# Lacadame/DiffSci

Measured on AMD Instinct MI355X. Metric: samples/sec (50-step Karras Heun), PUNetG 64ch 128x128, higher is better.
Workload: dtype f32 (3x3 convs: fp16 hi+lo split, 3 fp16 MFMA products, fp32 accumulate); 1 GPU; PUNetG 64-base-ch, 1x128x128 fields, batch 64 per GPU, 50-step Heun deterministic sampler (99 network evaluations); global_batch=64, parallelism=dp1 (batch shards, all-gather of samples), world_size=1, backend=none (one process), hipgraph=True

## Files before the change

diffsci_amd/csrc/ds_attn3h.hip:

```cpp
#include <cstdlib>

#include "ds_common.h"
#include "ds_conv_epilogue.h"
#include "ds_h3_common.h"

namespace {

using ds::f32x4;
using ds::wave_max;
using ds_epi::f32x16;
using ds_h3::f16x8;
using ds_h3::split2;
using ds_h3::u32x4;
typedef unsigned u32x2 __attribute__((ext_vector_type(2)));

constexpr int NT = 256;
constexpr int KB = 32;
constexpr float RESCALE_T = 8.0f;

constexpr float LOG2E = 1.44269504088896341f;

__device__ __forceinline__ f16x8 as_f16x8(u32x4 v) { return __builtin_bit_cast(f16x8, v); }

template <int ET, bool IMG, bool MH>
__global__ __launch_bounds__(NT) void k_attn3h(float* out, const float* __restrict__ q, size_t q_bs,
                                               const u32x4* __restrict__ kimg, const u32x4* __restrict__ vimg, int L, int heads,
                                               float scale, float thr, const unsigned* q_amax, const unsigned* k_amax,
                                               const unsigned* v_amax, unsigned* out_amax) {
  constexpr int E = 32 * ET;
  constexpr int NDG = E / 8;
  constexpr int NS = E / 16;
  constexpr int KITEMS = NDG * KB;
  constexpr int KI = (KITEMS + NT - 1) / NT;
  constexpr int VITEMS = E * 4;
  constexpr int VI = (VITEMS + NT - 1) / NT;
  extern __shared__ __attribute__((aligned(16))) unsigned char smem[];
  constexpr int KVEC = 2 * NDG * KB;
  constexpr int VVEC = 2 * 4 * E;
  u32x4* Kbuf = reinterpret_cast<u32x4*>(smem);
  u32x4* Vbuf = Kbuf + 2 * KVEC;
  const int tid = threadIdx.x, lane = tid & 63;
  const int wv = __builtin_amdgcn_readfirstlane(tid >> 6);
  const int li = lane & 31, lh = lane >> 5;
  unsigned qblk, b_u;
  {
    const unsigned nx = gridDim.x;
    const unsigned id = blockIdx.x + nx * blockIdx.y;
    const unsigned total = nx * gridDim.y;
    const unsigned per = total >> 3, rem = total & 7u;
    const unsigned xcd = id & 7u, k = id >> 3;
    const unsigned logical = xcd * per + (xcd < rem ? xcd : rem) + k;
    qblk = logical % nx;
    b_u = logical / nx;
  }
  const int row = (int)b_u;
  const int b = MH ? row / heads : row, h = MH ? row - b * heads : 0;
  const int Etot = MH ? E * heads : E;
  const int q0_raw = ((int)qblk * 4 + wv) * 32;
  const bool active = q0_raw < L;
  const int q0 = active ? q0_raw : L - 32;
  const float* Qt = q + (size_t)b * q_bs + (size_t)h * E * L;
  const float* Kt = Qt + (size_t)Etot * L;
  const float* Vt = Kt + (size_t)Etot * L;
  const unsigned q_bits = ds_epi::act_bits(q_amax, b), k_bits = ds_epi::act_bits(k_amax, b), v_bits = ds_epi::act_bits(v_amax, b);
  const int aq = ds_epi::act_exponent_of(q_bits, -60, 60);
  const int ak = ds_epi::act_exponent_of(k_bits, -60, 60);
  const int av = ds_epi::act_exponent_of(v_bits, -120, 120);
  const float a_in = ds_epi::pow2f(ak), v_in = ds_epi::pow2f(av);
  const float s_un = ds_epi::pow2f(-(aq + ak)), o_un = ds_epi::pow2f(-av);
  scale = ds_epi::mul_pow2(scale, aq);

  u32x4 qh[NS], ql[NS];
#pragma unroll
  for (int s = 0; s < NS; ++s) {
    float v[8];
#pragma unroll
    for (int k = 0; k < 8; ++k)
      v[k] = Qt[(size_t)(16 * s + 8 * lh + k) * L + q0 + li] * scale;
#pragma unroll
    for (int k = 0; k < 4; ++k) {
      unsigned h, l;
      split2(v[2 * k], v[2 * k + 1], h, l);
      qh[s][k] = h; ql[s][k] = l;
    }
  }

  f32x16 O[ET];
#pragma unroll
  for (int t = 0; t < ET; ++t)
#pragma unroll
    for (int r = 0; r < 16; ++r) O[t][r] = 0.f;
  float m_run = -INFINITY, l_run = 0.f;

  static_assert(KI * 8 == VI * 8, "K and V staging share one register set");
  float sr[KI][8];
  unsigned koff[KI], voff[VI];
#pragma unroll
  for (int i = 0; i < KI; ++i) {
    const int e = tid + NT * i;
    const int dg = (e / KB) % NDG, key = e % KB;
    koff[i] = (unsigned)(8 * dg) * (unsigned)L + (unsigned)key;
  }
#pragma unroll
  for (int i = 0; i < VI; ++i) {
    const int e = tid + NT * i;
    const int d = (e >> 2) % E, kg = e & 3;
    voff[i] = (unsigned)d * (unsigned)L + (unsigned)(8 * kg);
  }
  auto k_load = [&](int key0) {
#pragma unroll
    for (int k = 0; k < 8; ++k) {
      const float* row = Kt + (size_t)k * L + key0;
#pragma unroll
      for (int i = 0; i < KI; ++i) sr[i][k] = row[koff[i]];
    }
  };
  auto k_store = [&](u32x4* Ks) {
#pragma unroll
    for (int i = 0; i < KI; ++i) {
      const int e = tid + NT * i;
      if (NT * (i + 1) <= KITEMS || e < KITEMS) {
        u32x4 h, l;
#pragma unroll
        for (int k = 0; k < 4; ++k) {
          unsigned a, c;
          split2(sr[i][2 * k] * a_in, sr[i][2 * k + 1] * a_in, a, c);
          h[k] = a; l[k] = c;
        }
        Ks[e] = h;
        Ks[NDG * KB + e] = l;
      }
    }
  };
  auto v_load = [&](int key0) {
    const float* base = Vt + key0;
#pragma unroll
    for (int i = 0; i < VI; ++i) {
      const float* p = base + voff[i];
      const f32x4 v0 = *reinterpret_cast<const f32x4*>(p);
      const f32x4 v1 = *reinterpret_cast<const f32x4*>(p + 4);
#pragma unroll
      for (int k = 0; k < 4; ++k) { sr[i][k] = v0[k]; sr[i][4 + k] = v1[k]; }
    }
  };
  auto v_store = [&](u32x4* Vs) {
#pragma unroll
    for (int i = 0; i < VI; ++i) {
      const int e = tid + NT * i;
      if (NT * (i + 1) <= VITEMS || e < VITEMS) {
        const int d = e >> 2, kg = e & 3;
        u32x4 h, l;
#pragma unroll
        for (int k = 0; k < 4; ++k) {
          unsigned a, c;
          split2(sr[i][2 * k] * v_in, sr[i][2 * k + 1] * v_in, a, c);
          h[k] = a; l[k] = c;
        }
        Vs[kg * E + d] = h;
        Vs[4 * E + kg * E + d] = l;
      }
    }
  };

  const int nkb = L / KB;
  static_assert(KVEC == VVEC && KVEC % (64 * 4) == 0, "image tiles are whole LDS-DMA pieces per wave");
  const u32x4* kimg_b = IMG ? kimg + (size_t)row * nkb * KVEC : nullptr;
  const u32x4* vimg_b = IMG ? vimg + (size_t)row * nkb * VVEC : nullptr;
  auto dma = [&](u32x4* dst, const u32x4* src) __attribute__((always_inline)) {
#pragma unroll
    for (int i = 0; i < KVEC / 256; ++i) {
      const int k = wv + 4 * i;
      __builtin_amdgcn_global_load_lds((const __attribute__((address_space(1))) void*)(src + 64 * k + lane),
                                       (__attribute__((address_space(3))) void*)(dst + 64 * k), 16, 0, 0);
    }
  };
  auto qk = [&](const u32x4* Ks) __attribute__((always_inline)) {
    f32x16 S, S1;
#pragma unroll
    for (int r = 0; r < 16; ++r) { S[r] = 0.f; S1[r] = 0.f; }
#pragma unroll
    for (int s = 0; s < NS; s += 2) {
      const f16x8 ah = as_f16x8(Ks[(2 * s + lh) * KB + li]);
      const f16x8 al = as_f16x8(Ks[NDG * KB + (2 * s + lh) * KB + li]);
      const f16x8 bh = as_f16x8(Ks[(2 * s + 2 + lh) * KB + li]);
      const f16x8 bl = as_f16x8(Ks[NDG * KB + (2 * s + 2 + lh) * KB + li]);
      S = __builtin_amdgcn_mfma_f32_32x32x16_f16(al, as_f16x8(qh[s]), S, 0, 0, 0);
      S1 = __builtin_amdgcn_mfma_f32_32x32x16_f16(bl, as_f16x8(qh[s + 1]), S1, 0, 0, 0);
      S = __builtin_amdgcn_mfma_f32_32x32x16_f16(ah, as_f16x8(ql[s]), S, 0, 0, 0);
      S1 = __builtin_amdgcn_mfma_f32_32x32x16_f16(bh, as_f16x8(ql[s + 1]), S1, 0, 0, 0);
      S = __builtin_amdgcn_mfma_f32_32x32x16_f16(ah, as_f16x8(qh[s]), S, 0, 0, 0);
      S1 = __builtin_amdgcn_mfma_f32_32x32x16_f16(bh, as_f16x8(qh[s + 1]), S1, 0, 0, 0);
    }
    return S + S1;
  };
  if constexpr (IMG) {
    dma(Kbuf, kimg_b);
    dma(Vbuf, vimg_b);
    if (nkb > 1) dma(Kbuf + KVEC, kimg_b + KVEC);
    asm volatile("s_waitcnt vmcnt(0)" ::: "memory");
    __syncthreads();
    f32x16 S = qk(Kbuf);
    for (int kb = 0; kb < nkb; ++kb) {
      const u32x4* Vs = Vbuf + (kb & 1) * VVEC;
      if (kb + 2 < nkb) dma(Kbuf + (kb & 1) * KVEC, kimg_b + (size_t)(kb + 2) * KVEC);
      if (kb + 1 < nkb) dma(Vbuf + ((kb + 1) & 1) * VVEC, vimg_b + (size_t)(kb + 1) * VVEC);
      f32x16 Sn;
      if (kb + 1 < nkb) Sn = qk(Kbuf + ((kb + 1) & 1) * KVEC);
      float mx = S[0];
#pragma unroll
      for (int r = 1; r < 16; ++r) mx = fmaxf(mx, S[r]);
      mx = fmaxf(mx, __shfl_xor(mx, 32, 64)) * s_un;
      if (__any(mx > m_run + thr)) {
        const float m_new = fmaxf(m_run, mx);
        const float alpha = expf(m_run - m_new);
        l_run = l_run * alpha;
        m_run = m_new;
#pragma unroll
        for (int t = 0; t < ET; ++t)
#pragma unroll
          for (int r = 0; r < 16; ++r) O[t][r] *= alpha;
      }
      float rs = 0.f;
      const float mneg = -m_run;
#pragma unroll
      for (int r = 0; r < 16; ++r) {
        S[r] = __builtin_amdgcn_exp2f(__builtin_fmaf(S[r], s_un, mneg) * LOG2E);
        rs += S[r];
      }
      rs += __shfl_xor(rs, 32, 64);
      l_run = l_run + rs;
      u32x4 ph[2], pl[2];
#pragma unroll
      for (int t = 0; t < 2; ++t) {
        unsigned h[4], l[4];
#pragma unroll
        for (int k = 0; k < 4; ++k) split2(S[8 * t + 2 * k], S[8 * t + 2 * k + 1], h[k], l[k]);
#pragma unroll
        for (int k = 0; k < 2; ++k) {
          u32x2 r = __builtin_amdgcn_permlane32_swap(h[k], h[2 + k], false, false);
          h[k] = r[0]; h[2 + k] = r[1];
          r = __builtin_amdgcn_permlane32_swap(l[k], l[2 + k], false, false);
          l[k] = r[0]; l[2 + k] = r[1];
        }
        ph[t] = u32x4{h[0], h[1], h[2], h[3]};
        pl[t] = u32x4{l[0], l[1], l[2], l[3]};
      }
#pragma unroll
      for (int t = 0; t < ET; ++t) {
#pragma unroll
        for (int sl = 0; sl < 2; ++sl) {
          const f16x8 vh = as_f16x8(Vs[(2 * sl + lh) * E + 32 * t + li]);
          const f16x8 vl = as_f16x8(Vs[4 * E + (2 * sl + lh) * E + 32 * t + li]);
          O[t] = __builtin_amdgcn_mfma_f32_32x32x16_f16(vl, as_f16x8(ph[sl]), O[t], 0, 0, 0);
          O[t] = __builtin_amdgcn_mfma_f32_32x32x16_f16(vh, as_f16x8(pl[sl]), O[t], 0, 0, 0);
          O[t] = __builtin_amdgcn_mfma_f32_32x32x16_f16(vh, as_f16x8(ph[sl]), O[t], 0, 0, 0);
        }
        if ((t & 1) == 1) __builtin_amdgcn_sched_barrier(0);
      }
      if (kb + 1 < nkb) S = Sn;
      asm volatile("s_waitcnt vmcnt(0)" ::: "memory");
      __syncthreads();
    }
  } else {
  if (IMG) {
    dma(Kbuf, kimg_b);
    dma(Vbuf, vimg_b);
  } else {
    k_load(0);
    k_store(Kbuf);
    v_load(0);
    v_store(Vbuf);
  }
  if (IMG) asm volatile("s_waitcnt vmcnt(0)" ::: "memory");
  __syncthreads();
  for (int kb = 0; kb < nkb; ++kb) {
    const bool more = kb + 1 < nkb;
    const u32x4* Ks = Kbuf + (kb & 1) * KVEC;
    const u32x4* Vs = Vbuf + (kb & 1) * VVEC;
    u32x4* Kn = Kbuf + ((kb + 1) & 1) * KVEC;
    u32x4* Vn = Vbuf + ((kb + 1) & 1) * VVEC;
    if (IMG) {
      if (more) { dma(Kn, kimg_b + (size_t)(kb + 1) * KVEC); dma(Vn, vimg_b + (size_t)(kb + 1) * VVEC); }
    } else if (more) {
      k_load((kb + 1) * KB);
    }
    f32x16 S;
    {
      f32x16 S1;
#pragma unroll
      for (int r = 0; r < 16; ++r) { S[r] = 0.f; S1[r] = 0.f; }
#pragma unroll
      for (int s = 0; s < NS; s += 2) {
        const f16x8 ah = as_f16x8(Ks[(2 * s + lh) * KB + li]);
        const f16x8 al = as_f16x8(Ks[NDG * KB + (2 * s + lh) * KB + li]);
        const f16x8 bh = as_f16x8(Ks[(2 * s + 2 + lh) * KB + li]);
        const f16x8 bl = as_f16x8(Ks[NDG * KB + (2 * s + 2 + lh) * KB + li]);
        S = __builtin_amdgcn_mfma_f32_32x32x16_f16(al, as_f16x8(qh[s]), S, 0, 0, 0);
        S1 = __builtin_amdgcn_mfma_f32_32x32x16_f16(bl, as_f16x8(qh[s + 1]), S1, 0, 0, 0);
        S = __builtin_amdgcn_mfma_f32_32x32x16_f16(ah, as_f16x8(ql[s]), S, 0, 0, 0);
        S1 = __builtin_amdgcn_mfma_f32_32x32x16_f16(bh, as_f16x8(ql[s + 1]), S1, 0, 0, 0);
        S = __builtin_amdgcn_mfma_f32_32x32x16_f16(ah, as_f16x8(qh[s]), S, 0, 0, 0);
        S1 = __builtin_amdgcn_mfma_f32_32x32x16_f16(bh, as_f16x8(qh[s + 1]), S1, 0, 0, 0);
        if ((s & 2) == 2) __builtin_amdgcn_sched_barrier(0);
      }
      S = S + S1;
    }
    if (!IMG && more) {
      k_store(Kn);
      v_load((kb + 1) * KB);
    }
    {
      float mx = S[0];
#pragma unroll
      for (int r = 1; r < 16; ++r) mx = fmaxf(mx, S[r]);
      mx = fmaxf(mx, __shfl_xor(mx, 32, 64)) * s_un;
      if (__any(mx > m_run + thr)) {
        const float m_new = fmaxf(m_run, mx);
        const float alpha = expf(m_run - m_new);
        l_run = l_run * alpha;
        m_run = m_new;
#pragma unroll
        for (int t = 0; t < ET; ++t)
#pragma unroll
          for (int r = 0; r < 16; ++r) O[t][r] *= alpha;
      }
      float rs = 0.f;
      const float mneg = -m_run;
#pragma unroll
      for (int r = 0; r < 16; ++r) {
        S[r] = __builtin_amdgcn_exp2f(__builtin_fmaf(S[r], s_un, mneg) * LOG2E);
        rs += S[r];
      }
      rs += __shfl_xor(rs, 32, 64);
      l_run = l_run + rs;
      u32x4 ph[2], pl[2];
#pragma unroll
      for (int t = 0; t < 2; ++t) {
        unsigned h[4], l[4];
#pragma unroll
        for (int k = 0; k < 4; ++k) split2(S[8 * t + 2 * k], S[8 * t + 2 * k + 1], h[k], l[k]);
#pragma unroll
        for (int k = 0; k < 2; ++k) {
          u32x2 r = __builtin_amdgcn_permlane32_swap(h[k], h[2 + k], false, false);
          h[k] = r[0]; h[2 + k] = r[1];
          r = __builtin_amdgcn_permlane32_swap(l[k], l[2 + k], false, false);
          l[k] = r[0]; l[2 + k] = r[1];
        }
        ph[t] = u32x4{h[0], h[1], h[2], h[3]};
        pl[t] = u32x4{l[0], l[1], l[2], l[3]};
      }
#pragma unroll
      for (int t = 0; t < ET; ++t) {
#pragma unroll
        for (int sl = 0; sl < 2; ++sl) {
          const f16x8 vh = as_f16x8(Vs[(2 * sl + lh) * E + 32 * t + li]);
          const f16x8 vl = as_f16x8(Vs[4 * E + (2 * sl + lh) * E + 32 * t + li]);
          O[t] = __builtin_amdgcn_mfma_f32_32x32x16_f16(vl, as_f16x8(ph[sl]), O[t], 0, 0, 0);
          O[t] = __builtin_amdgcn_mfma_f32_32x32x16_f16(vh, as_f16x8(pl[sl]), O[t], 0, 0, 0);
          O[t] = __builtin_amdgcn_mfma_f32_32x32x16_f16(vh, as_f16x8(ph[sl]), O[t], 0, 0, 0);
        }
        if ((t & 1) == 1) __builtin_amdgcn_sched_barrier(0);
      }
    }
    if (!IMG && more) v_store(Vn);
    if (IMG) asm volatile("s_waitcnt vmcnt(0)" ::: "memory");
    __syncthreads();
  }
  }
  float amax = 0.f;
  if (active) {
    const float inv = (1.0f / l_run) * o_un;
    float* ob = out + ((size_t)b * Etot + (size_t)h * E) * L;
#pragma unroll
    for (int t = 0; t < ET; ++t)
#pragma unroll
      for (int r = 0; r < 16; ++r) {
        const int d = 32 * t + (r & 3) + 8 * (r >> 2) + 4 * lh;
        const float o = O[t][r] * inv;
        ob[(size_t)d * L + q0 + li] = o;
        amax = fmaxf(amax, __builtin_fabsf(o));
      }
  }
  if (out_amax) ds::wave_commit_max_always(out_amax + b, amax);
}

template <int ET, bool MH>
__global__ __launch_bounds__(NT) void k_attn_images(u32x4* __restrict__ kimg, u32x4* __restrict__ vimg,
                                                   const float* __restrict__ ksrc, size_t k_bs, const float* __restrict__ vsrc,
                                                   size_t v_bs, int L, int heads, const unsigned* k_amax, const unsigned* v_amax) {
  constexpr int E = 32 * ET, NDG = E / 8;
  constexpr int KITEMS = NDG * KB, VITEMS = E * 4;
  const int tid = threadIdx.x, kb = blockIdx.x, row = blockIdx.y, nkb = L / KB;
  const int b = MH ? row / heads : row, h = MH ? row - b * heads : 0;
  const float a_in = ds_epi::pow2f(ds_epi::act_exponent_of(ds_epi::act_bits(k_amax, b), -60, 60));
  const float v_in = ds_epi::pow2f(ds_epi::act_exponent_of(ds_epi::act_bits(v_amax, b), -120, 120));
  const float* Kt = ksrc + (size_t)b * k_bs + (size_t)h * E * L + (size_t)kb * KB;
  const float* Vt = vsrc + (size_t)b * v_bs + (size_t)h * E * L + (size_t)kb * KB;
  u32x4* Kd = kimg + ((size_t)row * nkb + kb) * (2 * KITEMS);
  u32x4* Vd = vimg + ((size_t)row * nkb + kb) * (2 * VITEMS);
  for (int e = tid; e < KITEMS; e += NT) {
    const int dg = e / KB, key = e % KB;
    u32x4 h, l;
#pragma unroll
    for (int k = 0; k < 4; ++k) {
      unsigned a, c;
      split2(Kt[(size_t)(8 * dg + 2 * k) * L + key] * a_in, Kt[(size_t)(8 * dg + 2 * k + 1) * L + key] * a_in, a, c);
      h[k] = a; l[k] = c;
    }
    Kd[e] = h;
    Kd[KITEMS + e] = l;
  }
  for (int e = tid; e < VITEMS; e += NT) {
    const int d = e >> 2, kg = e & 3;
    const float* p = Vt + (size_t)d * L + 8 * kg;
    const f32x4 v0 = *reinterpret_cast<const f32x4*>(p) * v_in, v1 = *reinterpret_cast<const f32x4*>(p + 4) * v_in;
    u32x4 h, l;
    unsigned a, c;
    split2(v0[0], v0[1], a, c); h[0] = a; l[0] = c;
    split2(v0[2], v0[3], a, c); h[1] = a; l[1] = c;
    split2(v1[0], v1[1], a, c); h[2] = a; l[2] = c;
    split2(v1[2], v1[3], a, c); h[3] = a; l[3] = c;
    Vd[kg * E + d] = h;
    Vd[VITEMS + kg * E + d] = l;
  }
}

struct AttnSrc {
  const float *q, *k, *v;
  size_t q_bs, k_bs, v_bs;
  const unsigned *q_amax, *k_amax, *v_amax;
};
AttnSrc qkv_src(const float* qkv, int B, int Etot, int L, const unsigned* in_amax) {
  const size_t third = (size_t)Etot * L;
  return AttnSrc{qkv, qkv + third, qkv + 2 * third, 3 * third, 3 * third, 3 * third, in_amax, in_amax, in_amax ? in_amax + B : nullptr};
}

template <int ET, bool IMG, bool MH>
int launch_attn3h(float* out, const AttnSrc& a, void* workspace, int B, int heads, int L, float scale, unsigned* out_amax,
                  hipStream_t s) {
  constexpr int E = 32 * ET;
  const size_t lds = (size_t)2 * (2 * (E / 8) * KB + 2 * 4 * E) * 16;
  if (lds > 48 * 1024) {
    const int rc = ds::ensure_dynamic_lds<&k_attn3h<ET, IMG, MH>>((int)lds, "hipFuncSetAttribute(attn3h)");
    if (rc != DS_OK) return rc;
  }
  const int rows = B * heads;
  u32x4* kimg = nullptr;
  u32x4* vimg = nullptr;
  if (IMG) {
    kimg = reinterpret_cast<u32x4*>(workspace);
    vimg = kimg + (size_t)rows * L * (E / 4);
    hipLaunchKernelGGL((k_attn_images<ET, MH>), dim3(L / KB, rows), dim3(NT), 0, s, kimg, vimg, a.k, a.k_bs, a.v, a.v_bs, L, heads,
                       a.k_amax, a.v_amax);
    DS_CHECK_LAUNCH("ds_attention_h3 (images)");
  }
  dim3 g((L + 127) / 128, rows);
  hipLaunchKernelGGL((k_attn3h<ET, IMG, MH>), g, dim3(NT), lds, s, out, a.q, a.q_bs, kimg, vimg, L, heads, scale, RESCALE_T,
                     a.q_amax, a.k_amax, a.v_amax, out_amax);
  DS_CHECK_LAUNCH("ds_attention_h3");
  return DS_OK;
}

template <bool IMG>
int attention_h3_src(float* out, const AttnSrc& a, void* workspace, int B, int E, int L, unsigned* out_amax, hipStream_t s) {
  const float scale = (float)sqrt(1.0 / (double)E);
  switch (E) {
    case 32: return launch_attn3h<1, IMG, false>(out, a, workspace, B, 1, L, scale, out_amax, s);
    case 64: return launch_attn3h<2, IMG, false>(out, a, workspace, B, 1, L, scale, out_amax, s);
    case 128: return launch_attn3h<4, IMG, false>(out, a, workspace, B, 1, L, scale, out_amax, s);
    case 256: return launch_attn3h<8, IMG, false>(out, a, workspace, B, 1, L, scale, out_amax, s);
    default:
      ds::set_error("ds_attention_h3: E=%d unsupported (32, 64, 128, 256)", E);
      return DS_ERR_UNSUPPORTED;
  }
}

template <bool IMG>
int attention_h3(float* out, const float* qkv, void* workspace, int B, int E, int L, const unsigned* in_amax, unsigned* out_amax,
                 void* stream) {
  DS_REQUIRE(out && qkv, DS_ERR_NULL, "ds_attention_h3: NULL pointer");
  DS_REQUIRE(B >= 0 && E > 0 && L > 0, DS_ERR_SHAPE, "ds_attention_h3: bad shape B=%d E=%d L=%d", B, E, L);
  DS_REQUIRE(L % 32 == 0, DS_ERR_UNSUPPORTED, "ds_attention_h3: L=%d must be a multiple of 32", L);
  DS_REQUIRE(B < 65536 && L / 32 < 65536 * 32, DS_ERR_SHAPE, "ds_attention_h3: B=%d exceeds grid.y", B);
  DS_REQUIRE((reinterpret_cast<uintptr_t>(qkv) & 15u) == 0, DS_ERR_SHAPE, "ds_attention_h3: qkv must be 16-byte aligned");
  DS_REQUIRE(!IMG || (workspace && (reinterpret_cast<uintptr_t>(workspace) & 15u) == 0), DS_ERR_NULL,
             "ds_attention_h3_ws: a 16-byte aligned workspace of ds_attention_h3_workspace_bytes(B, E, L) bytes is required");
  if (B == 0) return DS_OK;
  return attention_h3_src<IMG>(out, qkv_src(qkv, B, E, L, in_amax), workspace, B, E, L, out_amax, ds::as_stream(stream));
}

bool mfma_head_width(int d) { return d == 32 || d == 64 || d == 128 || d == 256; }

__global__ __launch_bounds__(64) void k_attn_heads_generic(float* out, const float* __restrict__ qkv, int d, int heads, int L,
                                                           float scale) {
  extern __shared__ float sm[];
  float* qs = sm;
  float* ps = sm + d;
  const int q = blockIdx.x, row = blockIdx.y, lane = threadIdx.x;
  const int b = row / heads, h = row - b * heads, Etot = d * heads;
  const float* Qt = qkv + ((size_t)b * 3 * Etot + (size_t)h * d) * L;
  const float* Kt = Qt + (size_t)Etot * L;
  const float* Vt = Kt + (size_t)Etot * L;
  for (int c = lane; c < d; c += 64) qs[c] = Qt[(size_t)c * L + q] * scale;
  __syncthreads();
  float mx = -INFINITY;
  for (int k = lane; k < L; k += 64) {
    float sc = 0.f;
    for (int c = 0; c < d; ++c) sc = fmaf(qs[c], Kt[(size_t)c * L + k], sc);
    ps[k] = sc;
    mx = fmaxf(mx, sc);
  }
  mx = wave_max(mx);
  float sum = 0.f;
  for (int k = lane; k < L; k += 64) {
    const float p = expf(ps[k] - mx);
    ps[k] = p;
    sum += p;
  }
  for (int o = 32; o > 0; o >>= 1) sum += __shfl_xor(sum, o, 64);
  __syncthreads();
  const float inv = 1.0f / sum;
  float* ob = out + ((size_t)b * Etot + (size_t)h * d) * L;
  for (int c = 0; c < d; ++c) {
    const float* v = Vt + (size_t)c * L;
    float acc = 0.f;
    for (int k = lane; k < L; k += 64) acc = fmaf(ps[k], v[k], acc);
    for (int o = 32; o > 0; o >>= 1) acc += __shfl_xor(acc, o, 64);
    if (lane == 0) ob[(size_t)c * L + q] = acc * inv;
  }
}

int heads_generic(float* out, const float* qkv, int B, int E, int heads, int L, hipStream_t s) {
  const int d = E / heads;
  const size_t lds = (size_t)(d + L) * sizeof(float);
  DS_REQUIRE(lds <= 64 * 1024, DS_ERR_UNSUPPORTED, "ds_attention_heads_generic: d + L = %d is too large for the generic path", d + L);
  if (B == 0) return DS_OK;
  if (lds > 48 * 1024) {
    const int rc = ds::ensure_dynamic_lds<&k_attn_heads_generic>(64 * 1024, "hipFuncSetAttribute(attn_heads_generic)");
    if (rc != DS_OK) return rc;
  }
  const float scale = (float)sqrt(1.0 / (double)d);
  hipLaunchKernelGGL(k_attn_heads_generic, dim3(L, B * heads), dim3(64), lds, s, out, qkv, d, heads, L, scale);
  DS_CHECK_LAUNCH("ds_attention_heads_generic");
  return DS_OK;
}

}

extern "C" int ds_attention_h3(float* out, const float* qkv, int B, int E, int L, const unsigned* in_amax, unsigned* out_amax,
                               void* stream) {
  return attention_h3<false>(out, qkv, nullptr, B, E, L, in_amax, out_amax, stream);
}

extern "C" size_t ds_attention_h3_workspace_bytes(int B, int E, int L) {
  if (B <= 0 || E <= 0 || L <= 0) return 0;
  return (size_t)B * L * E * 8;
}

extern "C" int ds_attention_h3_ws(float* out, const float* qkv, void* workspace, int B, int E, int L, const unsigned* in_amax,
                                  unsigned* out_amax, void* stream) {
  return attention_h3<true>(out, qkv, workspace, B, E, L, in_amax, out_amax, stream);
}

extern "C" int ds_attention_h3_xkv(float* out, const float* q, const float* x, void* workspace, int B, int E, int L,
                                   const unsigned* q_amax, const unsigned* k_amax, const unsigned* v_amax, unsigned* out_amax,
                                   void* stream, int flags) {
  DS_REQUIRE(out && q && x, DS_ERR_NULL, "ds_attention_h3_xkv: NULL pointer");
  DS_REQUIRE(flags == 0, DS_ERR_UNSUPPORTED, "ds_attention_h3_xkv: flags=%d must be 0", flags);
  DS_REQUIRE(B >= 0 && E > 0 && L > 0, DS_ERR_SHAPE, "ds_attention_h3_xkv: bad shape B=%d E=%d L=%d", B, E, L);
  DS_REQUIRE(L % 32 == 0, DS_ERR_UNSUPPORTED, "ds_attention_h3_xkv: L=%d must be a multiple of 32", L);
  DS_REQUIRE(B < 65536 && L / 32 < 65536 * 32, DS_ERR_SHAPE, "ds_attention_h3_xkv: B=%d exceeds grid.y", B);
  DS_REQUIRE(((reinterpret_cast<uintptr_t>(q) | reinterpret_cast<uintptr_t>(x)) & 15u) == 0, DS_ERR_SHAPE,
             "ds_attention_h3_xkv: q and x must be 16-byte aligned");
  DS_REQUIRE(workspace && (reinterpret_cast<uintptr_t>(workspace) & 15u) == 0, DS_ERR_NULL,
             "ds_attention_h3_xkv: a 16-byte aligned workspace of ds_attention_h3_workspace_bytes(B, E, L) bytes is required");
  if (B == 0) return DS_OK;
  const size_t bs = (size_t)E * L;
  return attention_h3_src<true>(out, AttnSrc{q, x, x, bs, bs, bs, q_amax, k_amax, v_amax}, workspace, B, E, L, out_amax,
                                ds::as_stream(stream));
}

extern "C" size_t ds_attention_h3_heads_workspace_bytes(int B, int E, int heads, int L) {
  if (B <= 0 || E <= 0 || L <= 0 || heads <= 0 || E % heads || !mfma_head_width(E / heads) || L % 32) return 0;
  return (size_t)B * L * E * 8;
}

extern "C" int ds_attention_h3_heads(float* out, const float* qkv, void* workspace, int B, int E, int heads, int L,
                                     const unsigned* in_amax, unsigned* out_amax, void* stream) {
  DS_REQUIRE(out && qkv, DS_ERR_NULL, "ds_attention_h3_heads: NULL pointer");
  DS_REQUIRE(B >= 0 && E > 0 && L > 0 && heads > 0, DS_ERR_SHAPE, "ds_attention_h3_heads: bad shape B=%d E=%d heads=%d L=%d",
             B, E, heads, L);
  DS_REQUIRE(E % heads == 0, DS_ERR_SHAPE, "ds_attention_h3_heads: E=%d is not a multiple of heads=%d", E, heads);
  DS_REQUIRE((size_t)B * heads < 65536, DS_ERR_SHAPE, "ds_attention_h3_heads: B*heads=%lld exceeds grid.y", (long long)B * heads);
  if (heads == 1) {
    if (workspace) return attention_h3<true>(out, qkv, workspace, B, E, L, in_amax, out_amax, stream);
    return attention_h3<false>(out, qkv, nullptr, B, E, L, in_amax, out_amax, stream);
  }
  if (B == 0) return DS_OK;
  const int d = E / heads;
  const float scale = (float)sqrt(1.0 / (double)d);
  hipStream_t s = ds::as_stream(stream);
  if (!mfma_head_width(d) || L % 32) {
    DS_REQUIRE(out_amax == nullptr, DS_ERR_UNSUPPORTED,
               "ds_attention_h3_heads: out_amax needs a head width in {32, 64, 128, 256} and L a multiple of 32 (reduce with "
               "ds_absmax_rows instead)");
    return heads_generic(out, qkv, B, E, heads, L, s);
  }
  DS_REQUIRE((reinterpret_cast<uintptr_t>(qkv) & 15u) == 0, DS_ERR_SHAPE, "ds_attention_h3_heads: qkv must be 16-byte aligned");
  DS_REQUIRE(!workspace || (reinterpret_cast<uintptr_t>(workspace) & 15u) == 0, DS_ERR_SHAPE,
             "ds_attention_h3_heads: the workspace must be 16-byte aligned");
  const bool img = workspace != nullptr;
  const AttnSrc a = qkv_src(qkv, B, E, L, in_amax);
  switch (d) {
    case 32: return img ? launch_attn3h<1, true, true>(out, a, workspace, B, heads, L, scale, out_amax, s)
                        : launch_attn3h<1, false, true>(out, a, nullptr, B, heads, L, scale, out_amax, s);
    case 64: return img ? launch_attn3h<2, true, true>(out, a, workspace, B, heads, L, scale, out_amax, s)
                        : launch_attn3h<2, false, true>(out, a, nullptr, B, heads, L, scale, out_amax, s);
    case 128: return img ? launch_attn3h<4, true, true>(out, a, workspace, B, heads, L, scale, out_amax, s)
                         : launch_attn3h<4, false, true>(out, a, nullptr, B, heads, L, scale, out_amax, s);
    default: return img ? launch_attn3h<8, true, true>(out, a, workspace, B, heads, L, scale, out_amax, s)
                        : launch_attn3h<8, false, true>(out, a, nullptr, B, heads, L, scale, out_amax, s);
  }
}

extern "C" int ds_attention_heads_generic(float* out, const float* qkv, int B, int E, int heads, int L, void* stream) {
  DS_REQUIRE(out && qkv, DS_ERR_NULL, "ds_attention_heads_generic: NULL pointer");
  DS_REQUIRE(B >= 0 && E > 0 && L > 0 && heads > 0, DS_ERR_SHAPE, "ds_attention_heads_generic: bad shape B=%d E=%d heads=%d L=%d",
             B, E, heads, L);
  DS_REQUIRE(E % heads == 0, DS_ERR_SHAPE, "ds_attention_heads_generic: E=%d is not a multiple of heads=%d", E, heads);
  DS_REQUIRE((size_t)B * heads < 65536, DS_ERR_SHAPE, "ds_attention_heads_generic: B*heads=%lld exceeds grid.y",
             (long long)B * heads);
  return heads_generic(out, qkv, B, E, heads, L, ds::as_stream(stream));
}
```

Measured before the change: 84.05 samples/s.

## Interleave softmax and LDS-DMA pieces under next-tile QK MFMAs in attention

Restructures the image-path attention loop so the softmax exponentials, hi/lo split and permlane swaps of the current tile, plus per-group LDS-DMA issue, run in slots between the next tile's QK^T MFMA groups. K and V fragments are software-pipelined through register double/triple buffers, and the next tile's max is computed right after the first PV MFMAs. The O rescale uses inline-asm accvgpr read/mul/write with explicit nops and is marked unlikely. This aims to hide VALU and DMA latency behind matrix-core work, at the cost of more registers, hand-tuned scheduling barriers and fragile inline asm.

```diff
diff --git a/diffsci_amd/csrc/ds_attn3h.hip b/diffsci_amd/csrc/ds_attn3h.hip
--- a/diffsci_amd/csrc/ds_attn3h.hip
+++ b/diffsci_amd/csrc/ds_attn3h.hip
@@ -166,32 +166,59 @@
   static_assert(KVEC == VVEC && KVEC % (64 * 4) == 0, "image tiles are whole LDS-DMA pieces per wave");
   const u32x4* kimg_b = IMG ? kimg + (size_t)row * nkb * KVEC : nullptr;
   const u32x4* vimg_b = IMG ? vimg + (size_t)row * nkb * VVEC : nullptr;
+  static_assert(KVEC / 256 == ET, "one LDS-DMA piece per wave, operand and group of the S^T product");
+  auto dma_piece = [&](u32x4* dst, const u32x4* src, int i) __attribute__((always_inline)) {
+    const int k = wv + 4 * i;
+    __builtin_amdgcn_global_load_lds((const __attribute__((address_space(1))) void*)(src + 64 * k + lane),
+                                     (__attribute__((address_space(3))) void*)(dst + 64 * k), 16, 0, 0);
+  };
   auto dma = [&](u32x4* dst, const u32x4* src) __attribute__((always_inline)) {
 #pragma unroll
-    for (int i = 0; i < KVEC / 256; ++i) {
-      const int k = wv + 4 * i;
-      __builtin_amdgcn_global_load_lds((const __attribute__((address_space(1))) void*)(src + 64 * k + lane),
-                                       (__attribute__((address_space(3))) void*)(dst + 64 * k), 16, 0, 0);
-    }
-  };
-  auto qk = [&](const u32x4* Ks) __attribute__((always_inline)) {
-    f32x16 S, S1;
-#pragma unroll
-    for (int r = 0; r < 16; ++r) { S[r] = 0.f; S1[r] = 0.f; }
+    for (int i = 0; i < ET; ++i) dma_piece(dst, src, i);
+  };
+  auto qk = [&](const u32x4* Ks, f32x16& S0, f32x16& S1, auto&& under) __attribute__((always_inline)) {
+    f16x8 fr[2][4];
+    auto frags = [&](int s, f16x8* f) __attribute__((always_inline)) {
+      f[0] = as_f16x8(Ks[(2 * s + lh) * KB + li]);
+      f[1] = as_f16x8(Ks[NDG * KB + (2 * s + lh) * KB + li]);
+      f[2] = as_f16x8(Ks[(2 * s + 2 + lh) * KB + li]);
+      f[3] = as_f16x8(Ks[NDG * KB + (2 * s + 2 + lh) * KB + li]);
+    };
+#pragma unroll
+    for (int r = 0; r < 16; ++r) { S0[r] = 0.f; S1[r] = 0.f; }
+    frags(0, fr[0]);
 #pragma unroll
     for (int s = 0; s < NS; s += 2) {
-      const f16x8 ah = as_f16x8(Ks[(2 * s + lh) * KB + li]);
-      const f16x8 al = as_f16x8(Ks[NDG * KB + (2 * s + lh) * KB + li]);
-      const f16x8 bh = as_f16x8(Ks[(2 * s + 2 + lh) * KB + li]);
-      const f16x8 bl = as_f16x8(Ks[NDG * KB + (2 * s + 2 + lh) * KB + li]);
-      S = __builtin_amdgcn_mfma_f32_32x32x16_f16(al, as_f16x8(qh[s]), S, 0, 0, 0);
+      const int g = s >> 1;
+      if (s + 2 < NS) frags(s + 2, fr[(g + 1) & 1]);
+      const f16x8 ah = fr[g & 1][0], al = fr[g & 1][1], bh = fr[g & 1][2], bl = fr[g & 1][3];
+      S0 = __builtin_amdgcn_mfma_f32_32x32x16_f16(al, as_f16x8(qh[s]), S0, 0, 0, 0);
       S1 = __builtin_amdgcn_mfma_f32_32x32x16_f16(bl, as_f16x8(qh[s + 1]), S1, 0, 0, 0);
-      S = __builtin_amdgcn_mfma_f32_32x32x16_f16(ah, as_f16x8(ql[s]), S, 0, 0, 0);
+      S0 = __builtin_amdgcn_mfma_f32_32x32x16_f16(ah, as_f16x8(ql[s]), S0, 0, 0, 0);
       S1 = __builtin_amdgcn_mfma_f32_32x32x16_f16(bh, as_f16x8(ql[s + 1]), S1, 0, 0, 0);
-      S = __builtin_amdgcn_mfma_f32_32x32x16_f16(ah, as_f16x8(qh[s]), S, 0, 0, 0);
+      S0 = __builtin_amdgcn_mfma_f32_32x32x16_f16(ah, as_f16x8(qh[s]), S0, 0, 0, 0);
       S1 = __builtin_amdgcn_mfma_f32_32x32x16_f16(bh, as_f16x8(qh[s + 1]), S1, 0, 0, 0);
-    }
-    return S + S1;
+      under(g);
+      __builtin_amdgcn_sched_barrier(0);
+    }
+  };
+  auto tile_max = [&](const f32x16& S) __attribute__((always_inline)) {
+    float mx = S[0];
+#pragma unroll
+    for (int r = 1; r < 16; ++r) mx = fmaxf(mx, S[r]);
+    return fmaxf(mx, __shfl_xor(mx, 32, 64)) * s_un;
+  };
+  auto rescale_O = [&](float alpha) __attribute__((always_inline)) {
+    asm volatile("s_nop 15\n\ts_nop 3" ::: "memory");
+#pragma unroll
+    for (int t = 0; t < ET; ++t)
+#pragma unroll
+      for (int r = 0; r < 16; ++r) {
+        float o = O[t][r], tmp;
+        asm volatile("v_accvgpr_read_b32 %1, %0\n\tv_mul_f32 %1, %1, %2\n\tv_accvgpr_write_b32 %0, %1" : "+a"(o), "=&v"(tmp) : "v"(alpha));
+        O[t][r] = o;
+      }
+    asm volatile("s_nop 3" ::: "memory");
   };
   if constexpr (IMG) {
     dma(Kbuf, kimg_b);
@@ -199,79 +226,92 @@
     if (nkb > 1) dma(Kbuf + KVEC, kimg_b + KVEC);
     asm volatile("s_waitcnt vmcnt(0)" ::: "memory");
     __syncthreads();
-    f32x16 S = qk(Kbuf);
-    for (int kb = 0; kb < nkb; ++kb) {
+    f32x16 S, Sn0, Sn1;
+    qk(Kbuf, Sn0, Sn1, [](int) {});
+    S = Sn0 + Sn1;
+    float mx = tile_max(S);
+    auto tile = [&](int kb, const bool last) __attribute__((always_inline)) {
       const u32x4* Vs = Vbuf + (kb & 1) * VVEC;
-      if (kb + 2 < nkb) dma(Kbuf + (kb & 1) * KVEC, kimg_b + (size_t)(kb + 2) * KVEC);
-      if (kb + 1 < nkb) dma(Vbuf + ((kb + 1) & 1) * VVEC, vimg_b + (size_t)(kb + 1) * VVEC);
-      f32x16 Sn;
-      if (kb + 1 < nkb) Sn = qk(Kbuf + ((kb + 1) & 1) * KVEC);
-      float mx = S[0];
-#pragma unroll
-      for (int r = 1; r < 16; ++r) mx = fmaxf(mx, S[r]);
-      mx = fmaxf(mx, __shfl_xor(mx, 32, 64)) * s_un;
-      if (__any(mx > m_run + thr)) {
+      u32x4* Kd = Kbuf + (kb & 1) * KVEC;
+      u32x4* Vd = Vbuf + ((kb + 1) & 1) * VVEC;
+      const u32x4* Kg = kimg_b + (size_t)min(kb + 2, nkb - 1) * KVEC;
+      const u32x4* Vg = vimg_b + (size_t)min(kb + 1, nkb - 1) * VVEC;
+      if (__builtin_expect(__any(mx > m_run + thr), 0)) {
         const float m_new = fmaxf(m_run, mx);
         const float alpha = expf(m_run - m_new);
         l_run = l_run * alpha;
         m_run = m_new;
-#pragma unroll
-        for (int t = 0; t < ET; ++t)
-#pragma unroll
-          for (int r = 0; r < 16; ++r) O[t][r] *= alpha;
+        rescale_O(alpha);
       }
       float rs = 0.f;
       const float mneg = -m_run;
-#pragma unroll
-      for (int r = 0; r < 16; ++r) {
-        S[r] = __builtin_amdgcn_exp2f(__builtin_fmaf(S[r], s_un, mneg) * LOG2E);
-        rs += S[r];
+      unsigned ph[2][4], pl[2][4];
+      auto softmax_step = [&](int i) __attribute__((always_inline)) {
+        if (i < 16) {
+          S[i] = __builtin_amdgcn_exp2f(__builtin_fmaf(S[i], s_un, mneg) * LOG2E);
+          rs += S[i];
+        } else {
+          const int t = (i - 16) >> 2, k = (i - 16) & 3;
+          split2(S[8 * t + 2 * k], S[8 * t + 2 * k + 1], ph[t][k], pl[t][k]);
+          if (k == 3) {
+#pragma unroll
+            for (int j = 0; j < 2; ++j) {
+              u32x2 r = __builtin_amdgcn_permlane32_swap(ph[t][j], ph[t][2 + j], false, false);
+              ph[t][j] = r[0]; ph[t][2 + j] = r[1];
+              r = __builtin_amdgcn_permlane32_swap(pl[t][j], pl[t][2 + j], false, false);
+              pl[t][j] = r[0]; pl[t][2 + j] = r[1];
+            }
+          }
+        }
+      };
+      constexpr int NI = 2 * ET;
+      f16x8 vf[3][2];
+      auto vfrags = [&](int i, f16x8* f) __attribute__((always_inline)) {
+        const int t = i >> 1, sl = i & 1;
+        f[0] = as_f16x8(Vs[(2 * sl + lh) * E + 32 * t + li]);
+        f[1] = as_f16x8(Vs[4 * E + (2 * sl + lh) * E + 32 * t + li]);
+      };
+      if (!last) {
+        qk(Kbuf + ((kb + 1) & 1) * KVEC, Sn0, Sn1, [&](int g) __attribute__((always_inline)) {
+#pragma unroll
+          for (int i = 24 * g / ET; i < 24 * (g + 1) / ET; ++i) softmax_step(i);
+          dma_piece(Kd, Kg, g);
+          dma_piece(Vd, Vg, g);
+          if (g == ET - 1) { vfrags(0, vf[0]); vfrags(1, vf[1]); }
+        });
+      } else {
+#pragma unroll
+        for (int i = 0; i < 24; ++i) softmax_step(i);
+        vfrags(0, vf[0]); vfrags(1, vf[1]);
       }
       rs += __shfl_xor(rs, 32, 64);
       l_run = l_run + rs;
-      u32x4 ph[2], pl[2];
-#pragma unroll
-      for (int t = 0; t < 2; ++t) {
-        unsigned h[4], l[4];
-#pragma unroll
-        for (int k = 0; k < 4; ++k) split2(S[8 * t + 2 * k], S[8 * t + 2 * k + 1], h[k], l[k]);
-#pragma unroll
-        for (int k = 0; k < 2; ++k) {
-          u32x2 r = __builtin_amdgcn_permlane32_swap(h[k], h[2 + k], false, false);
-          h[k] = r[0]; h[2 + k] = r[1];
-          r = __builtin_amdgcn_permlane32_swap(l[k], l[2 + k], false, false);
-          l[k] = r[0]; l[2 + k] = r[1];
+      const u32x4 ph0{ph[0][0], ph[0][1], ph[0][2], ph[0][3]}, pl0{pl[0][0], pl[0][1], pl[0][2], pl[0][3]};
+      const u32x4 ph1{ph[1][0], ph[1][1], ph[1][2], ph[1][3]}, pl1{pl[1][0], pl[1][1], pl[1][2], pl[1][3]};
+#pragma unroll
+      for (int i = 0; i < NI; ++i) {
+        if (i + 2 < NI) vfrags(i + 2, vf[(i + 2) % 3]);
+        const f16x8 vh = vf[i % 3][0], vl = vf[i % 3][1];
+        const f16x8 bh = as_f16x8((i & 1) ? ph1 : ph0), bl = as_f16x8((i & 1) ? pl1 : pl0);
+        O[i >> 1] = __builtin_amdgcn_mfma_f32_32x32x16_f16(vl, bh, O[i >> 1], 0, 0, 0);
+        O[i >> 1] = __builtin_amdgcn_mfma_f32_32x32x16_f16(vh, bl, O[i >> 1], 0, 0, 0);
+        O[i >> 1] = __builtin_amdgcn_mfma_f32_32x32x16_f16(vh, bh, O[i >> 1], 0, 0, 0);
+        if (!last && i == 1) {
+          S = Sn0 + Sn1;
+          mx = tile_max(S);
         }
-        ph[t] = u32x4{h[0], h[1], h[2], h[3]};
-        pl[t] = u32x4{l[0], l[1], l[2], l[3]};
-      }
-#pragma unroll
-      for (int t = 0; t < ET; ++t) {
-#pragma unroll
-        for (int sl = 0; sl < 2; ++sl) {
-          const f16x8 vh = as_f16x8(Vs[(2 * sl + lh) * E + 32 * t + li]);
-          const f16x8 vl = as_f16x8(Vs[4 * E + (2 * sl + lh) * E + 32 * t + li]);
-          O[t] = __builtin_amdgcn_mfma_f32_32x32x16_f16(vl, as_f16x8(ph[sl]), O[t], 0, 0, 0);
-          O[t] = __builtin_amdgcn_mfma_f32_32x32x16_f16(vh, as_f16x8(pl[sl]), O[t], 0, 0, 0);
-          O[t] = __builtin_amdgcn_mfma_f32_32x32x16_f16(vh, as_f16x8(ph[sl]), O[t], 0, 0, 0);
-        }
-        if ((t & 1) == 1) __builtin_amdgcn_sched_barrier(0);
-      }
-      if (kb + 1 < nkb) S = Sn;
+        __builtin_amdgcn_sched_barrier(0);
+      }
       asm volatile("s_waitcnt vmcnt(0)" ::: "memory");
       __syncthreads();
-    }
+    };
+    for (int kb = 0; kb + 1 < nkb; ++kb) tile(kb, false);
+    tile(nkb - 1, true);
   } else {
-  if (IMG) {
-    dma(Kbuf, kimg_b);
-    dma(Vbuf, vimg_b);
-  } else {
-    k_load(0);
-    k_store(Kbuf);
-    v_load(0);
-    v_store(Vbuf);
-  }
-  if (IMG) asm volatile("s_waitcnt vmcnt(0)" ::: "memory");
+  k_load(0);
+  k_store(Kbuf);
+  v_load(0);
+  v_store(Vbuf);
   __syncthreads();
   for (int kb = 0; kb < nkb; ++kb) {
     const bool more = kb + 1 < nkb;
@@ -279,11 +319,7 @@
     const u32x4* Vs = Vbuf + (kb & 1) * VVEC;
     u32x4* Kn = Kbuf + ((kb + 1) & 1) * KVEC;
     u32x4* Vn = Vbuf + ((kb + 1) & 1) * VVEC;
-    if (IMG) {
-      if (more) { dma(Kn, kimg_b + (size_t)(kb + 1) * KVEC); dma(Vn, vimg_b + (size_t)(kb + 1) * VVEC); }
-    } else if (more) {
-      k_load((kb + 1) * KB);
-    }
+    if (more) k_load((kb + 1) * KB);
     f32x16 S;
     {
       f32x16 S1;
@@ -310,19 +346,13 @@
       v_load((kb + 1) * KB);
     }
     {
-      float mx = S[0];
-#pragma unroll
-      for (int r = 1; r < 16; ++r) mx = fmaxf(mx, S[r]);
-      mx = fmaxf(mx, __shfl_xor(mx, 32, 64)) * s_un;
-      if (__any(mx > m_run + thr)) {
+      const float mx = tile_max(S);
+      if (__builtin_expect(__any(mx > m_run + thr), 0)) {
         const float m_new = fmaxf(m_run, mx);
         const float alpha = expf(m_run - m_new);
         l_run = l_run * alpha;
         m_run = m_new;
-#pragma unroll
-        for (int t = 0; t < ET; ++t)
-#pragma unroll
-          for (int r = 0; r < 16; ++r) O[t][r] *= alpha;
+        rescale_O(alpha);
       }
       float rs = 0.f;
       const float mneg = -m_run;
@@ -362,8 +392,7 @@
         if ((t & 1) == 1) __builtin_amdgcn_sched_barrier(0);
       }
     }
-    if (!IMG && more) v_store(Vn);
-    if (IMG) asm volatile("s_waitcnt vmcnt(0)" ::: "memory");
+    if (more) v_store(Vn);
     __syncthreads();
   }
   }
```

Result: faster. 84.92 samples/s, median of 6 (+1.0%).
